# sndels/yuki

Measured on AMD Instinct MI355X. Metric: Mray/s (primary+secondary), Path integrator @1080p, higher is better.
Workload: dtype f32; 1 GPU; cfg3: city 40x20 displaced icospheres, 1,024,012 triangles, SAH BVH (max_shapes_in_node 1), Path 8 bounces, Stratified 8x8, 1920x1080; triangles=1024012, spp=64, max_depth=8, tiles=8160, partition=single GPU, frames_in_flight=2

## Files before the change

### yuki_amd/csrc/yk_kernels.h

```cpp
#pragma once
#include <hip/hip_runtime.h>

#include "yk_device.h"

namespace yk {

unsigned trace_block_size();
unsigned trace_spill_depth();
unsigned trace_top_nodes();
unsigned trace_top_nodes_any();
unsigned packet_blocks_per_cu();
void launch_trace_closest_packet(hipStream_t s, unsigned grid, const DevScene& sc, const float4* rayO, const float4* rayD, const unsigned* count_ptr,
                                 unsigned* head, int* hit_tri, unsigned long long* ray_counter, const float4* lean_origin = nullptr, CancelRef cancel = CancelRef{nullptr, nullptr});
void launch_trace_any_packet(hipStream_t s, unsigned grid, const DevScene& sc, const ShadowQueue& q, unsigned char* vis, unsigned long long* shadow_counter,
                             CancelRef cancel = CancelRef{nullptr, nullptr});
unsigned trace_blocks_per_cu();

void launch_pixel_table(hipStream_t s, const yk_tile* tiles, const uint32_t* tile_offset, uint32_t n_tiles, uint32_t n_pixels, uint32_t* pixel_xy,
                        const uint16_t* tile_sample = nullptr, uint32_t* pixel_sample = nullptr);
void launch_pixel_table_one(hipStream_t s, const yk_tile& tile, uint32_t n_pixels, uint32_t* pixel_xy, uint32_t tile_sample, uint32_t* pixel_sample);
void launch_raygen(hipStream_t s, const DevCamera& cam, const RenderParams& prm, const uint32_t* pixel_xy, const uint32_t* pixel_sample, uint64_t work0,
                   uint32_t n, PathBuffers out, float4* sample_buf, unsigned* count, float4* lean_origin = nullptr, const uint4* pixel_aux = nullptr);
void launch_pixel_sampler(hipStream_t s, const SamplerCfg& cfg, const uint32_t* pixel_xy, uint32_t n_pixels, uint4* pixel_aux);
void launch_raygen_user(hipStream_t s, const RenderParams& prm, const float* o, const float* d, const uint16_t* pixel, const uint32_t* sample_index,
                        uint32_t dimension, uint32_t n, PathBuffers out, float4* sample_buf, uint32_t* pixel_xy, unsigned* ctrl);
void launch_trace_closest(hipStream_t s, unsigned grid, const DevScene& sc, const float4* rayO, const float4* rayD, const float* t_max_opt,
                          const unsigned* count_ptr, unsigned* head, int* hit_tri, float4* hit_out, uint4* stats_out, uint2* spill,
                          unsigned spill_stride, unsigned* ctrl, unsigned long long* ray_counter, const unsigned* cancel_host = nullptr);
void launch_whitted(hipStream_t s, unsigned grid, const DevScene& sc, const RenderParams& prm, const uint32_t* pixel_xy, const uint32_t* sample_index_tab,
                    PathBuffers cur, uint32_t n, float4* sample_buf, uint2* spill, unsigned spill_stride, unsigned* ctrl, unsigned long long* counters);
unsigned whitted_max_depth();
void launch_path_debug(hipStream_t s, unsigned grid, const DevScene& sc, const RenderParams& prm, const uint32_t* pixel_xy, const uint32_t* sample_index_tab,
                       PathBuffers cur, uint32_t n, float4* sample_buf, uint32_t* out_counts, float4* out_rays, unsigned ray_cap, uint32_t* out_n_rays,
                       float min_len, uint2* spill, unsigned spill_stride, unsigned* ctrl);
void launch_trace_any(hipStream_t s, unsigned grid, const DevScene& sc, const ShadowQueue& q, unsigned char* vis, uint2* spill, unsigned spill_stride,
                      unsigned* ctrl, unsigned long long* shadow_counter, const unsigned* cancel_host = nullptr);
void launch_shade(hipStream_t s, unsigned grid, const DevScene& sc, const RenderParams& prm, const uint32_t* pixel_xy, const uint32_t* sample_index_tab,
                  PathBuffers cur, PathBuffers nxt, const BounceQueues& q, unsigned split_delta, unsigned reorder, unsigned block_slots, unsigned sid_base,
                  const float4* lean_origin);
void launch_accumulate(hipStream_t s, unsigned grid, const RenderParams& prm, PathBuffers cur, const BounceQueues& q, unsigned nl, float4* sample_buf,
                       unsigned first, unsigned sid_base);
void launch_resolve(hipStream_t s, const float4* sample_buf, uint32_t n_pixels, uint32_t spp, float* out_rgb);
void launch_resolve_passes(hipStream_t s, const float4* sample_buf, uint32_t n_pixels, uint32_t n_passes, float* out_rgb, size_t pass_stride);
void launch_film_scatter(hipStream_t s, const uint32_t* pixel_xy, uint32_t n_pixels, const float* tile_rgb, uint32_t res_x, float* film_rgb, int accumulate,
                         uint32_t n_passes = 1, size_t pass_stride = 0);
void launch_debug_shade(hipStream_t s, const DevScene& sc, uint32_t integrator, PathBuffers cur, const int* hit_tri, const uint4* stats, uint32_t n,
                        float4* sample_buf);
void launch_guides(hipStream_t s, const DevScene& sc, PathBuffers cur, const int* hit_tri, uint32_t n, const uint32_t* pixel_xy, uint32_t res_x, float4* guides);
void launch_guides_ids(hipStream_t s, const DevScene& sc, PathBuffers cur, const int* hit_tri, uint32_t n, const uint32_t* pixel_xy, uint32_t res_x, float4* guides, uint4* ids);
void launch_ad_fold_samples(hipStream_t s, const uint32_t* pixel_xy, uint32_t n, const float4* sample_buf, uint32_t n_passes, uint32_t res_x, float* film_sum,
                            void* stats);
void launch_device_math(hipStream_t s, int fn, size_t n, const float* a, const float* b, float* out);
void launch_sampler_sequence(hipStream_t s, const SamplerCfg& cfg, uint32_t px, uint32_t py, uint32_t sample_index, const uint8_t* dims, size_t n_draws,
                             float* out);
void launch_light_test(hipStream_t s, const DevLight& L, int index, size_t n, const float* p, const float* ng, const float* u, float* out);
void launch_bsdf_test(hipStream_t s, const Material& m, size_t n, const float* ng, const float* ns, const float* dpdu, const float* wo,
                      const float* wi_or_u, int sample, float* out);
void launch_surface_test(hipStream_t s, const DevScene& sc, size_t n, const float4* rayO, const float4* rayD, const int* hit_word, int route, float* out);
void launch_pack_rays(hipStream_t s, size_t n, const float* o, const float* d, float4* rayO, float4* rayD);
void launch_pack_shadow_rays(hipStream_t s, size_t n, const float* o, const float* d, const float* t_max, const int* area_light, float4* shO,
                             float4* shD);
void launch_unpack_rays(hipStream_t s, size_t n, const float4* rayO, const float4* rayD, float* o, float* d);

}
```

### yuki_amd/csrc/yk_kernels.hip

```cpp
#include <hip/hip_runtime.h>

#include "yk_device.h"
#include "yk_geom.h"
#include "yk_kernels.h"
#include "yk_path_state.h"
#include "yk_rng.h"
#include "yk_shade.h"
#include "yk_shade_queue.h"
#include "yk_wave.h"

namespace yk {

__global__ void k_pixel_table(const yk_tile* tiles, const uint32_t* tile_offset, uint32_t n_tiles, uint32_t n_pixels,
                              uint32_t* pixel_xy, const uint16_t* tile_sample, uint32_t* pixel_sample) {
    uint32_t i = blockIdx.x * blockDim.x + threadIdx.x;
    if (i >= n_pixels) return;
    uint32_t lo = 0, hi = n_tiles;
    while (hi - lo > 1) {
        uint32_t mid = (lo + hi) >> 1;
        if (tile_offset[mid] <= i)
            lo = mid;
        else
            hi = mid;
    }
// ... 6 lines not shown
}

__global__ void k_pixel_table_one(yk_tile t, uint32_t n_pixels, uint32_t* pixel_xy, uint32_t tile_sample, uint32_t* pixel_sample) {
    uint32_t i = blockIdx.x * blockDim.x + threadIdx.x;
    if (i >= n_pixels) return;
    uint32_t w = (uint32_t)t.x1 - t.x0;
    pixel_xy[i] = (t.x0 + i % w) | ((t.y0 + i / w) << 16);
    if (pixel_sample) pixel_sample[i] = tile_sample;
}

__global__ void k_pixel_sampler(SamplerCfg cfg, const uint32_t* pixel_xy, uint32_t n_pixels, uint4* pixel_aux) {
    uint32_t i = blockIdx.x * blockDim.x + threadIdx.x;
    if (i >= n_pixels) return;
    const uint32_t xy = pixel_xy[i];
    const PixelSampler ps = pixel_sampler(cfg, xy & 0xffffu, xy >> 16);
    pixel_aux[i] = make_uint4((unsigned)ps.stream, (unsigned)(ps.stream >> 32), ps.hash0, 0u);
}

__device__ __forceinline__ void camera_ray(const DevCamera& cam, float fx, float fy, V3& o, V3& d) {
    V3 p_camera = xf_point(cam.r2c, V3{fx, fy, 0.0f});
    V3 dir = normalize(p_camera);
    o = xf_point(cam.c2w, V3{0.0f, 0.0f, 0.0f});
    d = xf_vector(cam.c2w, dir);
}

__global__ void k_raygen(DevCamera cam, RenderParams prm, const uint32_t* pixel_xy, const uint32_t* pixel_sample, uint64_t work0, uint32_t n,
                         PathBuffers out, float4* sample_buf, unsigned* count, float4* lean_origin, const uint4* pixel_aux) {
    uint32_t i = blockIdx.x * blockDim.x + threadIdx.x;
    if (cancel_raised(prm.cancel)) return;
    if (i == 0) *count = n;
    if (i >= n) return;
    const uint32_t w = (uint32_t)(work0 + i);
    uint32_t pix, ks;
    split_sample_id(w, prm.spe, pix, ks);
    const uint32_t s = (pixel_sample ? pixel_sample[pix] : prm.sample_base) + ks;
    uint32_t xy = pixel_xy[pix];
    uint32_t px = xy & 0xffffu, py = xy >> 16;
    SamplerState st;
    float ux, uy;
    if (pixel_aux) {
        const uint4 a = pixel_aux[pix];
        PixelSampler ps;
        ps.stream = (u64)a.x | ((u64)a.y << 32);
        ps.hash0 = a.z;
        st = sampler_start_camera(prm.sampler, ps, px, py, s, ux, uy);
    } else {
        st = sampler_start(prm.sampler, px, py, s, 0);
        sampler_get_2d(prm.sampler, st, ux, uy);
    }
    V3 o, d;
    camera_ray(cam, (float)px + ux, (float)py + uy, o, d);
    path_store_camera(out, i, o, d, w, st, lean_origin, i == 0);
    if (prm.integrator != YK_INTEGRATOR_PATH || prm.max_depth == 0) sample_buf[w] = make_float4(0.0f, 0.0f, 0.0f, 0.0f);
}

__global__ void k_raygen_user(RenderParams prm, const float* ray_o, const float* ray_d, const uint16_t* pixel, const uint32_t* sample_index,
                              uint32_t dimension, uint32_t n, PathBuffers out, float4* sample_buf, uint32_t* pixel_xy, unsigned* count) {
    uint32_t i = blockIdx.x * blockDim.x + threadIdx.x;
    if (i == 0) *count = n;
    if (i >= n) return;
    uint32_t px = pixel[2 * i], py = pixel[2 * i + 1];
    pixel_xy[i] = px | (py << 16);
    SamplerState st = sampler_start(prm.sampler, px, py, sample_index[i], dimension);
    if (prm.sampler.kind == 1) st.dimension = dimension;
    path_store_camera(out, i, ld3(ray_o, i), ld3(ray_d, i), i, st, nullptr, false);
    if (prm.integrator != YK_INTEGRATOR_PATH || prm.max_depth == 0) sample_buf[i] = make_float4(0.0f, 0.0f, 0.0f, 0.0f);
}

#ifdef YK_SHADE_PROFILE
#include "../../tools/micro/shade_profile.h"
#else
#define YK_PROF_DECL
#define YK_PROF_STAMP(k)
#define YK_PROF_FLUSH
#endif

template <int BLOCK, int CAP, int CAPQ>
__global__ __launch_bounds__(BLOCK, SHADE_MIN_WAVES) void k_shade(DevScene sc, RenderParams prm, const uint32_t* pixel_xy, const uint32_t* sample_index_tab,
                                                                  PathBuffers cur, PathBuffers nxt, BounceQueues q, ShadeArgs a,
                                                                  const float4* __restrict__ lean_origin) {
    static_assert(sizeof(ShadeStaging<CAP, CAPQ>) <= 53296, "k_shade: more LDS than the measured 53296 bytes per block (42 granules = 53760 cost the third block per CU)");
    __shared__ ShadeStaging<CAP, CAPQ> stg;
    const unsigned win_iters = min(a.win_max, max(1u, *q.count / (BLOCK * a.block_slots)));
    ShadeQueue<BLOCK, CAP, CAPQ> sq(stg, q, nxt, sc, a.split_delta);
    const unsigned n = sq.begin(prm.cancel);
    const unsigned WIN = win_iters * BLOCK;
    const unsigned n_win = (n + WIN - 1) / WIN;
    YK_PROF_DECL
    for (unsigned w = blockIdx.x; w < n_win; w += gridDim.x) {
        const unsigned wbase = w * WIN;
        YK_PROF_STAMP(0)
        const unsigned n_sub = a.reorder ? sort_window<BLOCK>(stg, q.hit, wbase, win_iters, n) : plain_window<BLOCK>(wbase, win_iters, n);
        for (unsigned sub = 0; sub < n_sub; ++sub) {
            const unsigned i = wbase + window_offset<BLOCK>(stg, a.reorder, sub);
            const bool valid = i < n;
            YK_PROF_STAMP(1)
            sq.room_for_iteration();
            PathState ps = path_inert();
            SamplerState st = sampler_inert();
            PathVertex v = vertex_inert();
            bool hit = false;
            if (valid) {
                ps = path_load(cur, i, lean_origin);
                st = path_sampler(prm, pixel_xy, sample_index_tab, ps);
                const int tri = q.hit[i];
                hit = tri >= 0;
                if (hit) vertex_setup(sc, (uint32_t)tri & YK_HIT_PRIM_MASK, ps.o, ps.d, v);
            }
            YK_PROF_STAMP(2)
            unsigned vword = 0u;
            for (unsigned l = 0; l < sq.nl; ++l) {
                NeeSample ne = nee_none();
                if (valid && hit) ne = vertex_light(sc, prm, st, l, v);
                sq.stage_shadow(ne, valid, i, l, vword);
            }
            sq.store_verdicts(valid, i, vword);
            YK_PROF_STAMP(3)
            bool alive = false;
            PathWords next = PathWords{make_float4(0, 0, 0, 0), make_float4(0, 0, 0, 0), make_float4(0, 0, 0, 0), make_uint4(0, 0, 0, 0)};
            if (valid) {
                unsigned kind = YK_PEND_MISS;
                RGB term = RGB{0, 0, 0};
                if (!hit) {
                    term = vertex_miss_term(sc, ps.beta);
                } else {
                    const VertexEnd e = vertex_finish(sc, prm, st, v, ps.beta, ps.bounces, ps.specular);
                    term = e.term;
                    kind = e.kind;
                    alive = e.alive;
                    if (e.sampled) {
                        ps.o = e.no;
                        ps.d = e.wi;
                        ps.dimension = st.dimension;
                        ps.rng = st.rng;
                        next = path_pack(ps);
                    }
                }
                q.pend[i] = pend_pack(term, kind, ps.sid - a.sid_base);
            }
            YK_PROF_STAMP(4)
            sq.stage_survivor(alive, next);
            YK_PROF_STAMP(5)
        }
        if (a.reorder) __syncthreads();
    }
    YK_PROF_FLUSH
    sq.finish();
}

__global__ void k_accumulate(RenderParams prm, PathBuffers cur, BounceQueues q, unsigned nl, float4* sample_buf, unsigned first, unsigned sid_base) {
    const unsigned n = cancel_raised(prm.cancel) ? 0u : *q.count;
    for (unsigned i = blockIdx.x * blockDim.x + threadIdx.x; i < n; i += gridDim.x * blockDim.x) {
        float4 p = q.pend[i];
        const unsigned kind = pend_kind(p);
        const unsigned sid = sid_base + pend_slot(p);
        RGB beta = RGB{1.0f, 1.0f, 1.0f};
        if (!first && !(kind & YK_PEND_MISS)) beta = path_beta(cur.thru[i]);
        RGB L = RGB{0.0f, 0.0f, 0.0f};
        if (!first) {
            const float4 acc = sample_buf[sid];
            L = RGB{acc.x, acc.y, acc.z};
        }
        RGB radiance = RGB{0.0f, 0.0f, 0.0f};
        if (!(kind & YK_PEND_MISS)) {
            const unsigned vs = YK_VIS_STRIDE(nl);
            const unsigned vword = vs == 4u ? reinterpret_cast<const unsigned*>(q.vis)[i] : 0u;
            for (unsigned l = 0; l < nl; ++l) {
// ... 70 lines not shown

__global__ void k_debug_shade(DevScene sc, uint32_t integrator, PathBuffers cur, const int* hit_tri, const uint4* stats, uint32_t n,
                              float4* sample_buf) {
    uint32_t i = blockIdx.x * blockDim.x + threadIdx.x;
    if (i >= n) return;
    const float4 rd = cur.rayD[i];
    int tri = hit_tri[i];
    RGB c = RGB{0.0f, 0.0f, 0.0f};
    if (integrator == YK_INTEGRATOR_BVH_INTERSECTIONS) {
        uint4 s = stats[i];
        c = RGB{(float)s.x, (float)s.y, tri >= 0 ? (float)s.y : 0.0f};
    } else if (tri >= 0 && integrator == YK_INTEGRATOR_SHADING_UVS) {
        Surface sf = hit_surface_prim(sc, (uint32_t)tri & YK_HIT_PRIM_MASK, f4_xyz(cur.rayO[i]), f4_xyz(rd), true);
        c = RGB{sf.u, sf.v, 0.0f};
    } else if (tri >= 0) {
        Surface sf = hit_surface_prim(sc, (uint32_t)tri & YK_HIT_PRIM_MASK, f4_xyz(cur.rayO[i]), f4_xyz(rd));
        V3 nn = integrator == YK_INTEGRATOR_GEOMETRY_NORMALS ? sf.n : sf.ns;
        c = RGB{nn.x, nn.y, nn.z} / 2.0f + 0.5f;
    }
    sample_buf[path_sample_id(rd)] = make_float4(c.r, c.g, c.b, 0.0f);
}

template <bool IDS>
__global__ void k_guides(DevScene sc, PathBuffers cur, const int* hit_tri, uint32_t n, const uint32_t* pixel_xy, uint32_t res_x, float4* guides, uint4* ids) {
    uint32_t i = blockIdx.x * blockDim.x + threadIdx.x;
    if (i >= n) return;
    const float4 rd = cur.rayD[i];
    const uint32_t xy = pixel_xy[path_sample_id(rd)];
    const size_t px = (size_t)(xy >> 16) * res_x + (xy & 0xffffu);
    const int tri = hit_tri[i];
    float4 a = make_float4(0.0f, 0.0f, 0.0f, 0.0f), b = a;
    uint4 id = make_uint4(YK_SURFACE_NONE, 0u, 0u, 0u);
    if (tri >= 0) {
        float t = 0.0f;
        const Surface sf = hit_surface_prim(sc, (uint32_t)tri & YK_HIT_PRIM_MASK, f4_xyz(cur.rayO[i]), f4_xyz(rd), sc.texels != nullptr, &t, IDS ? &id : nullptr);
        a = make_float4(sf.ns.x, sf.ns.y, sf.ns.z, 1.0f);
        b = make_float4(sf.p.x, sf.p.y, sf.p.z, t);
    }
    if (!IDS || guides) {
        guides[2 * px] = a;
        guides[2 * px + 1] = b;
    }
    if (IDS && ids) ids[px] = id;
}

#ifdef YK_SHADE_PROFILE
}
extern "C" int yk_debug_shade_profile(unsigned long long* out8, int reset) {
    unsigned long long zero[8] = {0, 0, 0, 0, 0, 0, 0, 0};
    (void)hipDeviceSynchronize();
    int rc = (int)hipMemcpyFromSymbol(out8, HIP_SYMBOL(yk::yk_shade_prof), sizeof(zero));
    if (reset) rc |= (int)hipMemcpyToSymbol(HIP_SYMBOL(yk::yk_shade_prof), zero, sizeof(zero));
    return rc;
}
namespace yk {
#endif

static inline unsigned blocks_for(size_t n, unsigned bs) { return (unsigned)((n + bs - 1) / bs); }

void launch_pixel_table(hipStream_t s, const yk_tile* tiles, const uint32_t* tile_offset, uint32_t n_tiles, uint32_t n_pixels, uint32_t* pixel_xy,
                        const uint16_t* tile_sample, uint32_t* pixel_sample) {
    if (!n_pixels) return;
    hipLaunchKernelGGL(k_pixel_table, dim3(blocks_for(n_pixels, 256)), dim3(256), 0, s, tiles, tile_offset, n_tiles, n_pixels, pixel_xy, tile_sample,
                       pixel_sample);
}
void launch_pixel_table_one(hipStream_t s, const yk_tile& tile, uint32_t n_pixels, uint32_t* pixel_xy, uint32_t tile_sample, uint32_t* pixel_sample) {
    if (!n_pixels) return;
    hipLaunchKernelGGL(k_pixel_table_one, dim3(blocks_for(n_pixels, 256)), dim3(256), 0, s, tile, n_pixels, pixel_xy, tile_sample, pixel_sample);
}
void launch_pixel_sampler(hipStream_t s, const SamplerCfg& cfg, const uint32_t* pixel_xy, uint32_t n_pixels, uint4* pixel_aux) {
    if (!n_pixels) return;
    hipLaunchKernelGGL(k_pixel_sampler, dim3(blocks_for(n_pixels, 256)), dim3(256), 0, s, cfg, pixel_xy, n_pixels, pixel_aux);
}
void launch_raygen(hipStream_t s, const DevCamera& cam, const RenderParams& prm, const uint32_t* pixel_xy, const uint32_t* pixel_sample, uint64_t work0,
                   uint32_t n, PathBuffers out, float4* sample_buf, unsigned* count, float4* lean_origin, const uint4* pixel_aux) {
    hipLaunchKernelGGL(k_raygen, dim3(blocks_for(n, 256)), dim3(256), 0, s, cam, prm, pixel_xy, pixel_sample, work0, n, out, sample_buf, count, lean_origin, pixel_aux);
}
void launch_raygen_user(hipStream_t s, const RenderParams& prm, const float* o, const float* d, const uint16_t* pixel, const uint32_t* sample_index,
                        uint32_t dimension, uint32_t n, PathBuffers out, float4* sample_buf, uint32_t* pixel_xy, unsigned* ctrl) {
    hipLaunchKernelGGL(k_raygen_user, dim3(blocks_for(n, 256)), dim3(256), 0, s, prm, o, d, pixel, sample_index, dimension, n, out, sample_buf,
                       pixel_xy, ctrl);
}
void launch_shade(hipStream_t s, unsigned grid, const DevScene& sc, const RenderParams& prm, const uint32_t* pixel_xy, const uint32_t* sample_index_tab,
                  PathBuffers cur, PathBuffers nxt, const BounceQueues& q, unsigned split_delta, unsigned reorder, unsigned block_slots, unsigned sid_base,
                  const float4* lean_origin) {
    const ShadeArgs a{split_delta, reorder, (unsigned)SHADE_WIN, block_slots, sid_base};
    hipLaunchKernelGGL((k_shade<256, SHADE_CAP, SHADE_CAPQ>), dim3(grid), dim3(256), 0, s, sc, prm, pixel_xy, sample_index_tab, cur, nxt, q, a, lean_origin);
}
void launch_accumulate(hipStream_t s, unsigned grid, const RenderParams& prm, PathBuffers cur, const BounceQueues& q, unsigned nl, float4* sample_buf,
                       unsigned first, unsigned sid_base) {
    hipLaunchKernelGGL(k_accumulate, dim3(grid), dim3(256), 0, s, prm, cur, q, nl, sample_buf, first, sid_base);
}
void launch_resolve(hipStream_t s, const float4* sample_buf, uint32_t n_pixels, uint32_t spp, float* out_rgb) {
    if (!n_pixels) return;
    hipLaunchKernelGGL(k_resolve, dim3(blocks_for(n_pixels, 256)), dim3(256), 0, s, sample_buf, n_pixels, spp, out_rgb);
}
void launch_resolve_passes(hipStream_t s, const float4* sample_buf, uint32_t n_pixels, uint32_t n_passes, float* out_rgb, size_t pass_stride) {
    if (!n_pixels) return;
    hipLaunchKernelGGL(k_resolve_passes, dim3(blocks_for((size_t)n_pixels * n_passes, 256)), dim3(256), 0, s, sample_buf, n_pixels, n_passes, out_rgb, pass_stride);
}
void launch_film_scatter(hipStream_t s, const uint32_t* pixel_xy, uint32_t n_pixels, const float* tile_rgb, uint32_t res_x, float* film_rgb, int accumulate,
                         uint32_t n_passes, size_t pass_stride) {
    if (!n_pixels) return;
    hipLaunchKernelGGL(k_film_scatter, dim3(blocks_for(n_pixels, 256)), dim3(256), 0, s, pixel_xy, n_pixels, tile_rgb, res_x, film_rgb, accumulate, n_passes, pass_stride);
}
void launch_debug_shade(hipStream_t s, const DevScene& sc, uint32_t integrator, PathBuffers cur, const int* hit_tri, const uint4* stats, uint32_t n,
                        float4* sample_buf) {
    hipLaunchKernelGGL(k_debug_shade, dim3(blocks_for(n, 256)), dim3(256), 0, s, sc, integrator, cur, hit_tri, stats, n, sample_buf);
}
void launch_guides(hipStream_t s, const DevScene& sc, PathBuffers cur, const int* hit_tri, uint32_t n, const uint32_t* pixel_xy, uint32_t res_x, float4* guides) {
    hipLaunchKernelGGL(k_guides<false>, dim3(blocks_for(n, 256)), dim3(256), 0, s, sc, cur, hit_tri, n, pixel_xy, res_x, guides, (uint4*)nullptr);
}
void launch_guides_ids(hipStream_t s, const DevScene& sc, PathBuffers cur, const int* hit_tri, uint32_t n, const uint32_t* pixel_xy, uint32_t res_x, float4* guides, uint4* ids) {
    hipLaunchKernelGGL(k_guides<true>, dim3(blocks_for(n, 256)), dim3(256), 0, s, sc, cur, hit_tri, n, pixel_xy, res_x, guides, ids);
}

}
```

### yuki_amd/csrc/yk_render.cpp

```cpp
#include <hip/hip_runtime.h>

#include <algorithm>
#include <chrono>
#include <cstdio>
#include <cstdlib>
#include <cstring>
#include <memory>
#include <mutex>
#include <string>
#include <thread>
#include <vector>

#include "yk_adaptive.h"
#include "yk_albedo.h"
#include "yk_film_call.h"
#include "yk_render_plan.h"
#include "yk_staging.h"
#ifdef YK_EXPERIMENT_SORT
#include "../../tools/micro/ray_sort_experiment.h"
#endif
#ifdef YK_EXPERIMENT_GRAPH
#include "../../tools/micro/graph_replay_experiment.h"
#endif

// ... 45 lines not shown
    p.thru = ws.path[which][2].as<float4>();
    p.rngs = ws.path[which][3].as<uint4>();
    return p;
}

static BounceQueues bounce_queues(WorkSet& ws, unsigned b) {
    unsigned* bc = ws.ctrl.as<unsigned>() + YK_CTRL_BOUNCE(b);
    BounceQueues q;
    q.hit = ws.hit.as<int>();
    q.pend = ws.pend.as<float4>();
    q.shC = ws.shC.as<float4>();
    q.vis = ws.vis.as<unsigned char>();
    q.area = ShadowQueue{ws.shO.as<float4>(), ws.shD.as<float4>(), ws.shq.as<unsigned>(), bc + YK_CTRL_SHQ, bc + YK_CTRL_HEAD + 1};
    q.delta = ShadowQueue{ws.shO2.as<float4>(), ws.shD2.as<float4>(), ws.shq2.as<unsigned>(), bc + YK_CTRL_SHQ2, bc + YK_CTRL_HEAD + 2};
    q.count = bc;
    q.next_count = bc + YK_CTRL_STRIDE;
    q.closest_head = bc + YK_CTRL_HEAD;
    return q;
}

yk_status make_params(yk_context* ctx, const yk_sampler_desc* smp, const yk_integrator_desc* integ, RenderParams& prm) {
    if (!smp || !integ) return fail(ctx, YK_ERR_INVALID_ARGUMENT, "null sampler/integrator");
    std::memset(&prm, 0, sizeof(prm));
    prm.sampler.kind = smp->kind;
    prm.sampler.nx = smp->nx;
    prm.sampler.ny = smp->kind == YK_SAMPLER_UNIFORM ? 1 : smp->ny;
    prm.sampler.jitter = smp->jitter;
    prm.sampler.seed = smp->seed;
    if (smp->kind > 1 || prm.sampler.nx == 0 || prm.sampler.ny == 0) return fail(ctx, YK_ERR_INVALID_ARGUMENT, "bad sampler");
    uint64_t spp = (uint64_t)prm.sampler.nx * prm.sampler.ny;
    if (spp > 0xFFFFu) return fail(ctx, YK_ERR_INVALID_ARGUMENT, "samples per pixel exceed u16 (integrators/mod.rs:139)");
    prm.sampler.spp = (unsigned)spp;
    prm.spe = (unsigned)spp;
    prm.max_depth = integ->max_depth;
    prm.has_clamp = integ->has_clamp;
    prm.clamp = integ->indirect_clamp;
    prm.integrator = integ->kind;
    if (integ->kind == YK_INTEGRATOR_WHITTED && integ->max_depth > whitted_max_depth())
        return fail(ctx, YK_ERR_UNSUPPORTED, "Whitted: max_depth above 16 is not supported on the device");
    if (integ->kind > YK_INTEGRATOR_SHADING_UVS) return fail(ctx, YK_ERR_INVALID_ARGUMENT, "bad integrator kind");
    return YK_OK;
}


bool packet_kernel_traces_bounce(const yk_context* ctx, const yk_scene* scene, unsigned b) {
    return b < (unsigned)ctx->packet_bounces && scene->bvh->depth <= 64;
}

void run_bounces(yk_context* ctx, WorkSet& ws, hipStream_t st, const yk_scene* scene, const RenderParams& prm, const uint32_t* pixel_xy,
                        const uint32_t* sample_index_tab, float4* sample_buf, KernelTimer& kt, unsigned long long* counters, bool coherent,
                        uint32_t n_paths, uint32_t sid_base, bool lean_camera_bounce, uint32_t* n_shadow_launches) {
    unsigned* ctrl = ws.ctrl.as<unsigned>();
    unsigned* errblk = error_block(ctx);
    const DevScene ds = dev_scene_for(scene, n_paths);
    auto fit = [](unsigned full, uint64_t items) { return (unsigned)std::min<uint64_t>(full, std::max<uint64_t>(1, (items + 255) / 256)); };
    const uint64_t n_shadow_max = (uint64_t)n_paths * std::max(1u, scene->n_lights);
    const unsigned tg = fit(trace_grid(ctx), n_paths), tg_any = fit(trace_grid(ctx), n_shadow_max);
    const unsigned pg_full = (unsigned)ctx->n_cu * packet_blocks_per_cu();
    const unsigned pg = fit(pg_full, n_paths), pg_any = fit(pg_full, n_shadow_max);
    static const unsigned shade_bpc = std::getenv("YK_SHADE_BPC") ? (unsigned)std::atoi(std::getenv("YK_SHADE_BPC")) : 256u;
    const unsigned sg = fit((unsigned)ctx->n_cu * shade_bpc, n_paths);
    const unsigned spill_stride = trace_grid(ctx) * trace_block_size();
    unsigned cur = 0;
    const bool overlap = ctx->overlap_shadow != 0 && ws.side != nullptr;
    hipStream_t sb = overlap ? ws.side : st;
    for (unsigned b = 0; b < prm.max_depth; ++b) {
        PathBuffers pc = path_buffers(ws, (int)cur), pn = path_buffers(ws, (int)(cur ^ 1u));
        const bool packet = coherent && packet_kernel_traces_bounce(ctx, scene, b);
        const float4* lean_origin = (b == 0 && lean_camera_bounce) ? reinterpret_cast<const float4*>(ctrl + YK_CTRL_CAM_O) : nullptr;
        const bool packet_shadow = coherent && b < (unsigned)ctx->packet_shadow_bounces && scene->bvh->depth <= 64 && scene->n_delta_lights > 0;
        const bool split = packet_shadow && scene->n_lights > scene->n_delta_lights;
        const bool all_delta = packet_shadow && !split;
        BounceQueues q = bounce_queues(ws, b);
        int e = kt.begin(st);
        if (packet)
            launch_trace_closest_packet(st, pg, ds, lean_origin ? nullptr : pc.rayO, pc.rayD, q.count, q.closest_head, q.hit, counters, lean_origin, prm.cancel);
        else {
            launch_trace_closest(st, tg, ds, pc.rayO, pc.rayD, nullptr, q.count, q.closest_head, q.hit, nullptr, nullptr,
                                 ws.spill.as<uint2>(), spill_stride, errblk, counters, prm.cancel.host);
        }
        kt.end(e, 0, st);
        if (overlap && b > 0) (void)hipStreamWaitEvent(st, ws.ev_acc, 0);
        e = kt.begin(st);
        launch_shade(st, sg, ds, prm, pixel_xy, sample_index_tab, pc, pn, q, split ? 1u : 0u, (b > 0 && ctx->shade_reorder) ? 1u : 0u, 3u * (unsigned)ctx->n_cu,
                     sid_base, lean_origin);
        kt.end(e, 2, st);
#ifdef YK_EXPERIMENT_SORT
        YK_SORT_AFTER_SHADE
#endif
        if (overlap) {
            (void)hipEventRecord(ws.ev_shade, st);
            (void)hipStreamWaitEvent(sb, ws.ev_shade, 0);
        }
        e = kt.begin(sb);
        uint2* any_spill = (overlap ? ws.spill_side : ws.spill).as<uint2>();
        if (all_delta) {
            launch_trace_any_packet(sb, pg_any, ds, q.area, q.vis, counters + 1, prm.cancel);
        } else {
            launch_trace_any(sb, tg_any, ds, q.area, q.vis, any_spill, spill_stride, errblk, counters + 1, prm.cancel.host);
            if (split && n_shadow_launches) ++*n_shadow_launches;
            if (split)
                launch_trace_any_packet(sb, pg_any, ds, q.delta, q.vis, counters + 1, prm.cancel);
        }
        kt.end(e, 1, sb);
        if (n_shadow_launches) ++*n_shadow_launches;
        launch_accumulate(sb, sg, prm, pc, q, ds.n_lights, sample_buf, b == 0 ? 1u : 0u, sid_base);
        if (overlap) (void)hipEventRecord(ws.ev_acc, sb);
        if (kt.on && std::getenv("YK_DEBUG_BOUNCES")) {
            unsigned h[YK_CTRL_STRIDE + 1];
            (void)hipStreamSynchronize(st);
            (void)hipStreamSynchronize(sb);
            (void)hipMemcpy(h, q.count, sizeof(h), hipMemcpyDeviceToHost);
            float tt = 0, ts = 0, th = 0;
            (void)hipEventElapsedTime(&tt, ctx->ev_pool[kt.spans[0].back().first], ctx->ev_pool[kt.spans[0].back().second]);
            (void)hipEventElapsedTime(&ts, ctx->ev_pool[kt.spans[1].back().first], ctx->ev_pool[kt.spans[1].back().second]);
            (void)hipEventElapsedTime(&th, ctx->ev_pool[kt.spans[2].back().first], ctx->ev_pool[kt.spans[2].back().second]);
            std::fprintf(stderr, "bounce %u: rays %u trace %.3f ms (%.0f Mray/s) | shadow rays %u %.3f ms (%.0f Mray/s) | shade %.3f ms | survivors %u\n", b, h[0],
                         tt, h[0] / (tt * 1e3), h[YK_CTRL_SHQ] + h[YK_CTRL_SHQ2], ts, (h[YK_CTRL_SHQ] + h[YK_CTRL_SHQ2]) / (ts * 1e3), th, h[YK_CTRL_STRIDE]);
        }
        cur ^= 1u;
    }
    if (overlap) (void)hipStreamWaitEvent(st, ws.ev_acc, 0);
}

static double now_ms() { return std::chrono::duration<double, std::milli>(std::chrono::steady_clock::now().time_since_epoch()).count(); }
static const bool g_debug_cancel = std::getenv("YK_DEBUG_CANCEL") != nullptr;

static void raise_cancel(yk_context* ctx, bool from_render_thread = true) {
    if (!ctx->cancel_host) return;
    const double t0 = g_debug_cancel ? now_ms() : 0.0;
    ctx->cancel_raised.store(true, std::memory_order_release);
    __atomic_store_n(ctx->cancel_host, 1u, __ATOMIC_RELEASE);
    if (from_render_thread && !ctx->cancel_stream) ctx->want_cancel_stream = true;
    if (from_render_thread && ctx->cancel_stream && ctx->counters.p)
        (void)hipMemcpyAsync(error_block(ctx) + YK_CTRL_CANCELLED, ctx->cancel_host + 16, 4, hipMemcpyHostToDevice, ctx->cancel_stream);
    if (g_debug_cancel) std::fprintf(stderr, "[yk cancel] raise: %s, %.3f ms\n", ctx->cancel_stream ? "host word + device word" : "host word only (first interruption)", now_ms() - t0);
}

static yk_status clear_cancel(yk_context* ctx) {
    if (!ctx->cancel_host || !ctx->cancel_raised.load(std::memory_order_acquire)) return YK_OK;
    HIP_TRY(ctx, hipStreamSynchronize(ctx->stream));
    if (ctx->cancel_stream) HIP_TRY(ctx, hipStreamSynchronize(ctx->cancel_stream));
    for (WorkSet& w : ctx->ws) {
        if (w.stream && w.stream != ctx->stream) HIP_TRY(ctx, hipStreamSynchronize(w.stream));
        if (w.side) HIP_TRY(ctx, hipStreamSynchronize(w.side));
    }
    __atomic_store_n(ctx->cancel_host, 0u, __ATOMIC_RELEASE);
    ctx->cancel_raised.store(false, std::memory_order_release);
    if (ctx->want_cancel_stream && !ctx->cancel_stream) {
        if (hipStreamCreateWithFlags(&ctx->cancel_stream, hipStreamNonBlocking) != hipSuccess) ctx->cancel_stream = nullptr;
        ctx->want_cancel_stream = false;
    }
    return YK_OK;
}

static bool poll_until(yk_context* ctx, hipEvent_t done, yk_cancel_fn cancel, void* user) {
    while (hipEventQuery(done) == hipErrorNotReady) {
        if (cancel(user)) {
            raise_cancel(ctx);
            return true;
        }
        std::this_thread::sleep_for(std::chrono::microseconds(100));
    }
    return false;
}
static bool wait_polling(yk_context* ctx, hipEvent_t done, hipStream_t st, yk_cancel_fn cancel, void* user) {
    const bool fired = cancel ? poll_until(ctx, done, cancel, user) : false;
    (void)hipStreamSynchronize(st);
// ... 913 lines not shown
```

### yuki_amd/csrc/yk_shade_queue.h

```cpp
#pragma once
#include "yk_device.h"
#include "yk_path_state.h"
#include "yk_shade.h"
#include "yk_wave.h"

#ifndef SHADE_CAP
#define SHADE_CAP 335
#endif
#ifndef SHADE_CAPQ
#define SHADE_CAPQ 768
#endif
#ifndef SHADE_WIN
#define SHADE_WIN 8
#endif
#ifndef SHADE_MIN_WAVES
#define SHADE_MIN_WAVES 3
#endif

namespace yk {

template <int CAP, int CAPQ> struct ShadeStaging {
    float4 pO[CAP], pD[CAP], pT[CAP];
    uint4 pR[CAP];
    float4 qO[CAPQ], qD[CAPQ];
    unsigned qS[CAPQ];
    unsigned fill_p, fill_q, gbase;
    unsigned q_delta;
    unsigned cancel;
    unsigned bucket[8];
    unsigned short order[SHADE_WIN * 256];
};

struct ShadeArgs {
    unsigned split_delta;
    unsigned reorder;
    unsigned win_max;
    unsigned block_slots;
    unsigned sid_base;
};

__device__ __forceinline__ unsigned block_append(bool want, unsigned* lds_fill) {
    unsigned long long mask = __ballot(want);
    unsigned total = (unsigned)__popcll(mask);
    unsigned prefix = (unsigned)__popcll(mask & ((1ull << lane_id()) - 1ull));
    unsigned base = 0;
    if (total && lane_id() == 0) base = atomicAdd(lds_fill, total);
    base = __shfl(base, 0);
    return base + prefix;
}

template <int BLOCK, class Staging>
__device__ __forceinline__ unsigned sort_window(Staging& stg, const int* hit_tri, unsigned wbase, unsigned win_iters, unsigned n) {
    if (threadIdx.x < 8) stg.bucket[threadIdx.x] = 0;
    __syncthreads();
    unsigned key[SHADE_WIN], rank[SHADE_WIN];
#pragma unroll
    for (int k = 0; k < SHADE_WIN; ++k) {
        const unsigned i0 = wbase + k * BLOCK + threadIdx.x;
        const bool in = (unsigned)k < win_iters && i0 < n;
        const int t = in ? hit_tri[i0] : -1;
        key[k] = !in ? 7u : (t < 0 ? 6u : ((unsigned)t >> YK_HIT_KIND_SHIFT));
    }
#pragma unroll
    for (int k = 0; k < SHADE_WIN; ++k) {
        rank[k] = 0;
        if ((unsigned)k >= win_iters) continue;
        for (unsigned q = 0; q < 8; ++q) {
            const unsigned long long m = __ballot(key[k] == q);
            if (m == 0ull) continue;
            unsigned b0 = 0;
            if (lane_id() == 0) b0 = atomicAdd(&stg.bucket[q], (unsigned)__popcll(m));
            b0 = __shfl(b0, 0);
            if (key[k] == q) rank[k] = b0 + (unsigned)__popcll(m & ((1ull << lane_id()) - 1ull));
        }
    }
    __syncthreads();
    unsigned first[8], n_sub;
    {
        unsigned acc = 0;
        for (unsigned q = 0; q < 8; ++q) {
            first[q] = acc;
            acc += stg.bucket[q];
        }
        n_sub = (acc - stg.bucket[7] + BLOCK - 1) / BLOCK;
    }
#pragma unroll
    for (int k = 0; k < SHADE_WIN; ++k)
        if ((unsigned)k < win_iters) stg.order[first[key[k]] + rank[k]] = (unsigned short)(k * BLOCK + threadIdx.x);
    __syncthreads();
    return n_sub;
}
template <int BLOCK> __device__ __forceinline__ unsigned plain_window(unsigned wbase, unsigned win_iters, unsigned n) {
    const unsigned left = n - wbase;
    return left >= win_iters * BLOCK ? win_iters : (left + BLOCK - 1) / BLOCK;
}
template <int BLOCK, class Staging> __device__ __forceinline__ unsigned window_offset(const Staging& stg, unsigned reorder, unsigned sub) {
    return reorder ? (unsigned)stg.order[sub * BLOCK + threadIdx.x] : sub * BLOCK + threadIdx.x;
}

template <int BLOCK, int CAP, int CAPQ> struct ShadeQueue {
    ShadeStaging<CAP, CAPQ>& stg;
    const BounceQueues& q;
    const PathBuffers& nxt;
    const DevScene& sc;
    const unsigned nl, split_delta;
    const bool per_iter;

    __device__ __forceinline__ ShadeQueue(ShadeStaging<CAP, CAPQ>& stg_, const BounceQueues& q_, const PathBuffers& nxt_, const DevScene& sc_, unsigned split_delta_)
        : stg(stg_), q(q_), nxt(nxt_), sc(sc_), nl(sc_.n_lights), split_delta(split_delta_), per_iter(!split_delta_ && BLOCK * sc_.n_lights <= (unsigned)CAPQ) {}

    __device__ __forceinline__ unsigned begin(const CancelRef& cancel) {
        if (threadIdx.x == 0) {
            stg.fill_p = 0;
            stg.fill_q = 0;
            stg.q_delta = 0;
            stg.cancel = cancel_raised(cancel) ? 1u : 0u;
        }
        __syncthreads();
        return __builtin_amdgcn_readfirstlane((int)stg.cancel) ? 0u : *q.count;
    }

    __device__ __forceinline__ void flush_q(unsigned fill, unsigned delta) {
        if (threadIdx.x == 0) stg.gbase = atomicAdd(delta ? q.delta.count : q.area.count, fill);
        __syncthreads();
        const unsigned gb = stg.gbase;
        float4* dO = delta ? q.delta.O : q.area.O;
        float4* dD = delta ? q.delta.D : q.area.D;
        unsigned* dS = delta ? q.delta.slot : q.area.slot;
        for (unsigned k = threadIdx.x; k < fill; k += BLOCK) {
            dO[gb + k] = stg.qO[k];
            dD[gb + k] = stg.qD[k];
            dS[gb + k] = stg.qS[k];
        }
        __syncthreads();
        if (threadIdx.x == 0) stg.fill_q = 0;
        __syncthreads();
    }
    __device__ __forceinline__ void flush_p(unsigned fill) {
        if (threadIdx.x == 0) stg.gbase = atomicAdd(q.next_count, fill);
        __syncthreads();
        const unsigned gb = stg.gbase;
        for (unsigned k = threadIdx.x; k < fill; k += BLOCK) {
            nxt.rayO[gb + k] = stg.pO[k];
            nxt.rayD[gb + k] = stg.pD[k];
            nxt.thru[gb + k] = stg.pT[k];
            nxt.rngs[gb + k] = stg.pR[k];
        }
        __syncthreads();
        if (threadIdx.x == 0) stg.fill_p = 0;
        __syncthreads();
    }

    __device__ __forceinline__ void room_for_iteration() {
        if (!per_iter) return;
        __syncthreads();
        const unsigned fq = stg.fill_q, fp = stg.fill_p, staged = stg.q_delta;
        __syncthreads();
        if (fq && fq + BLOCK * nl > CAPQ) flush_q(fq, staged);
        if (fp + BLOCK > CAP) flush_p(fp);
    }
    __device__ __forceinline__ void room_for_light(unsigned l) {
        if (per_iter) return;
        __syncthreads();
        const unsigned f = stg.fill_q, staged = stg.q_delta;
        const unsigned delta = (split_delta && sc.lights[l].kind != YK_LIGHT_RECT) ? 1u : 0u;
        __syncthreads();
        if (f && (staged != delta || f + BLOCK > CAPQ)) flush_q(f, staged);
        if (threadIdx.x == 0) stg.q_delta = delta;
    }
    __device__ __forceinline__ void room_for_survivor() {
        if (per_iter) return;
        __syncthreads();
        const unsigned f = stg.fill_p;
        __syncthreads();
        if (f + BLOCK > CAP) flush_p(f);
    }

    __device__ __forceinline__ void stage_shadow(const NeeSample& ne, bool valid, unsigned i, unsigned l, unsigned& vword) {
        const unsigned vs = YK_VIS_STRIDE(nl);
        const unsigned slot = i * nl + l, vslot = i * vs + l;
        const bool want = ne.want;
        if (vs == 4u)
            vword |= (want ? 1u : 0u) << (8u * l);
        else if (valid)
            q.vis[vslot] = want ? 1 : 0;
        room_for_light(l);
        const unsigned k = block_append(want, &stg.fill_q);
        if (want) {
            stg.qO[k] = make_float4(ne.so.x, ne.so.y, ne.so.z, YK_SHADOW_T_MAX);
            stg.qD[k] = make_float4(ne.sd.x, ne.sd.y, ne.sd.z, __uint_as_float((unsigned)ne.al));
            stg.qS[k] = vslot;
            q.shC[slot] = make_float4(ne.contrib.r, ne.contrib.g, ne.contrib.b, 0.0f);
        }
    }
    __device__ __forceinline__ void store_verdicts(bool valid, unsigned i, unsigned vword) {
        if (YK_VIS_STRIDE(nl) == 4u && valid) reinterpret_cast<unsigned*>(q.vis)[i] = vword;
    }

    __device__ __forceinline__ void stage_survivor(bool alive, const PathWords& w) {
        room_for_survivor();
        const unsigned j = block_append(alive, &stg.fill_p);
        if (alive) {
            stg.pO[j] = w.O;
            stg.pD[j] = w.D;
            stg.pT[j] = w.T;
            stg.pR[j] = w.R;
        }
    }

    __device__ __forceinline__ void finish() {
        __syncthreads();
        const unsigned fq = stg.fill_q, fp = stg.fill_p;
        if (fq) flush_q(fq, stg.q_delta);
        if (fp) flush_p(fp);
    }
};

}
```

Before: 2283 Mray/s.

## Split shade shadow staging into per-class LDS regions with merged flushes

The shade kernel's shadow-ray staging buffer is split into separate area and delta regions sized by a host-computed plan, so the kernel no longer flushes whenever the light class changes. All three queues (survivors, area, delta) are flushed together in one barrier round, with their atomics issued from different waves. Survivor staging capacity drops from 335 to 256, which shrinks LDS use but can force survivor flushes more often. The per-iteration decision mode now depends on the light count fitting the region slots even when delta lights are split.

```diff
diff --git a/yuki_amd/csrc/yk_kernels.h b/yuki_amd/csrc/yk_kernels.h
--- a/yuki_amd/csrc/yk_kernels.h
+++ b/yuki_amd/csrc/yk_kernels.h
@@ -36,8 +36,8 @@
 void launch_trace_any(hipStream_t s, unsigned grid, const DevScene& sc, const ShadowQueue& q, unsigned char* vis, uint2* spill, unsigned spill_stride,
                       unsigned* ctrl, unsigned long long* shadow_counter, const unsigned* cancel_host = nullptr);
 void launch_shade(hipStream_t s, unsigned grid, const DevScene& sc, const RenderParams& prm, const uint32_t* pixel_xy, const uint32_t* sample_index_tab,
-                  PathBuffers cur, PathBuffers nxt, const BounceQueues& q, unsigned split_delta, unsigned reorder, unsigned block_slots, unsigned sid_base,
-                  const float4* lean_origin);
+                  PathBuffers cur, PathBuffers nxt, const BounceQueues& q, unsigned split_delta, unsigned n_area_lights, unsigned reorder,
+                  unsigned block_slots, unsigned sid_base, const float4* lean_origin);
 void launch_accumulate(hipStream_t s, unsigned grid, const RenderParams& prm, PathBuffers cur, const BounceQueues& q, unsigned nl, float4* sample_buf,
                        unsigned first, unsigned sid_base);
 void launch_resolve(hipStream_t s, const float4* sample_buf, uint32_t n_pixels, uint32_t spp, float* out_rgb);
diff --git a/yuki_amd/csrc/yk_kernels.hip b/yuki_amd/csrc/yk_kernels.hip
--- a/yuki_amd/csrc/yk_kernels.hip
+++ b/yuki_amd/csrc/yk_kernels.hip
@@ -112,7 +112,7 @@
     static_assert(sizeof(ShadeStaging<CAP, CAPQ>) <= 53296, "k_shade: more LDS than the measured 53296 bytes per block (42 granules = 53760 cost the third block per CU)");
     __shared__ ShadeStaging<CAP, CAPQ> stg;
     const unsigned win_iters = min(a.win_max, max(1u, *q.count / (BLOCK * a.block_slots)));
-    ShadeQueue<BLOCK, CAP, CAPQ> sq(stg, q, nxt, sc, a.split_delta);
+    ShadeQueue<BLOCK, CAP, CAPQ> sq(stg, q, nxt, sc, a);
     const unsigned n = sq.begin(prm.cancel);
     const unsigned WIN = win_iters * BLOCK;
     const unsigned n_win = (n + WIN - 1) / WIN;
@@ -349,9 +349,10 @@
                        pixel_xy, ctrl);
 }
 void launch_shade(hipStream_t s, unsigned grid, const DevScene& sc, const RenderParams& prm, const uint32_t* pixel_xy, const uint32_t* sample_index_tab,
-                  PathBuffers cur, PathBuffers nxt, const BounceQueues& q, unsigned split_delta, unsigned reorder, unsigned block_slots, unsigned sid_base,
-                  const float4* lean_origin) {
-    const ShadeArgs a{split_delta, reorder, (unsigned)SHADE_WIN, block_slots, sid_base};
+                  PathBuffers cur, PathBuffers nxt, const BounceQueues& q, unsigned split_delta, unsigned n_area_lights, unsigned reorder,
+                  unsigned block_slots, unsigned sid_base, const float4* lean_origin) {
+    const ShadeRegions regions = shade_regions(sc.n_lights, split_delta ? n_area_lights : sc.n_lights, (unsigned)SHADE_CAPQ, 256u);
+    const ShadeArgs a{split_delta, regions, reorder, (unsigned)SHADE_WIN, block_slots, sid_base};
     hipLaunchKernelGGL((k_shade<256, SHADE_CAP, SHADE_CAPQ>), dim3(grid), dim3(256), 0, s, sc, prm, pixel_xy, sample_index_tab, cur, nxt, q, a, lean_origin);
 }
 void launch_accumulate(hipStream_t s, unsigned grid, const RenderParams& prm, PathBuffers cur, const BounceQueues& q, unsigned nl, float4* sample_buf,
diff --git a/yuki_amd/csrc/yk_render.cpp b/yuki_amd/csrc/yk_render.cpp
--- a/yuki_amd/csrc/yk_render.cpp
+++ b/yuki_amd/csrc/yk_render.cpp
@@ -151,8 +151,8 @@
         kt.end(e, 0, st);
         if (overlap && b > 0) (void)hipStreamWaitEvent(st, ws.ev_acc, 0);
         e = kt.begin(st);
-        launch_shade(st, sg, ds, prm, pixel_xy, sample_index_tab, pc, pn, q, split ? 1u : 0u, (b > 0 && ctx->shade_reorder) ? 1u : 0u, 3u * (unsigned)ctx->n_cu,
-                     sid_base, lean_origin);
+        launch_shade(st, sg, ds, prm, pixel_xy, sample_index_tab, pc, pn, q, split ? 1u : 0u, scene->n_lights - scene->n_delta_lights,
+                     (b > 0 && ctx->shade_reorder) ? 1u : 0u, 3u * (unsigned)ctx->n_cu, sid_base, lean_origin);
         kt.end(e, 2, st);
 #ifdef YK_EXPERIMENT_SORT
         YK_SORT_AFTER_SHADE
diff --git a/yuki_amd/csrc/yk_shade_queue.h b/yuki_amd/csrc/yk_shade_queue.h
--- a/yuki_amd/csrc/yk_shade_queue.h
+++ b/yuki_amd/csrc/yk_shade_queue.h
@@ -2,10 +2,11 @@
 #include "yk_device.h"
 #include "yk_path_state.h"
 #include "yk_shade.h"
+#include "yk_shade_regions.h"
 #include "yk_wave.h"
 
 #ifndef SHADE_CAP
-#define SHADE_CAP 335
+#define SHADE_CAP 256
 #endif
 #ifndef SHADE_CAPQ
 #define SHADE_CAPQ 768
@@ -24,8 +25,9 @@
     uint4 pR[CAP];
     float4 qO[CAPQ], qD[CAPQ];
     unsigned qS[CAPQ];
-    unsigned fill_p, fill_q, gbase;
-    unsigned q_delta;
+    unsigned fill_p;
+    unsigned fill_q[2];
+    unsigned gbase_p, gbase_q[2];
     unsigned cancel;
     unsigned bucket[8];
     unsigned short order[SHADE_WIN * 256];
@@ -33,6 +35,7 @@
 
 struct ShadeArgs {
     unsigned split_delta;
+    ShadeRegions regions;
     unsigned reorder;
     unsigned win_max;
     unsigned block_slots;
@@ -99,81 +102,93 @@
 }
 
 template <int BLOCK, int CAP, int CAPQ> struct ShadeQueue {
+    static_assert(CAP >= BLOCK, "the survivor staging holds an iteration");
+    static_assert(CAPQ % BLOCK == 0 && CAPQ >= 2 * BLOCK, "shade_regions deals whole blocks, at least one per class");
+    static_assert(BLOCK >= 192, "flush: threads 0, 64 and 128 reserve");
     ShadeStaging<CAP, CAPQ>& stg;
     const BounceQueues& q;
     const PathBuffers& nxt;
     const DevScene& sc;
     const unsigned nl, split_delta;
     const bool per_iter;
-
-    __device__ __forceinline__ ShadeQueue(ShadeStaging<CAP, CAPQ>& stg_, const BounceQueues& q_, const PathBuffers& nxt_, const DevScene& sc_, unsigned split_delta_)
-        : stg(stg_), q(q_), nxt(nxt_), sc(sc_), nl(sc_.n_lights), split_delta(split_delta_), per_iter(!split_delta_ && BLOCK * sc_.n_lights <= (unsigned)CAPQ) {}
+    const unsigned delta_base;
+    const unsigned full_area, full_delta;
+
+    __device__ __forceinline__ ShadeQueue(ShadeStaging<CAP, CAPQ>& stg_, const BounceQueues& q_, const PathBuffers& nxt_, const DevScene& sc_, const ShadeArgs& a)
+        : stg(stg_), q(q_), nxt(nxt_), sc(sc_), nl(sc_.n_lights), split_delta(a.split_delta), per_iter(a.regions.one_decision != 0u),
+          delta_base(a.regions.delta_base),
+          full_area(room_left(a.regions.area_cap, per_iter ? a.regions.need_area : (unsigned)BLOCK)),
+          full_delta(room_left(a.regions.delta_cap, per_iter ? a.regions.need_delta : (unsigned)BLOCK)) {}
+    static __device__ __forceinline__ unsigned room_left(unsigned cap, unsigned need) { return cap > need ? cap - need : 0u; }
+
+    static __device__ __forceinline__ unsigned uniform(unsigned v) { return (unsigned)__builtin_amdgcn_readfirstlane((int)v); }
+    __device__ __forceinline__ unsigned light_class(unsigned l) const { return (split_delta && sc.lights[l].kind != YK_LIGHT_RECT) ? 1u : 0u; }
 
     __device__ __forceinline__ unsigned begin(const CancelRef& cancel) {
         if (threadIdx.x == 0) {
             stg.fill_p = 0;
-            stg.fill_q = 0;
-            stg.q_delta = 0;
+            stg.fill_q[0] = 0;
+            stg.fill_q[1] = 0;
             stg.cancel = cancel_raised(cancel) ? 1u : 0u;
         }
         __syncthreads();
-        return __builtin_amdgcn_readfirstlane((int)stg.cancel) ? 0u : *q.count;
-    }
-
-    __device__ __forceinline__ void flush_q(unsigned fill, unsigned delta) {
-        if (threadIdx.x == 0) stg.gbase = atomicAdd(delta ? q.delta.count : q.area.count, fill);
-        __syncthreads();
-        const unsigned gb = stg.gbase;
-        float4* dO = delta ? q.delta.O : q.area.O;
-        float4* dD = delta ? q.delta.D : q.area.D;
-        unsigned* dS = delta ? q.delta.slot : q.area.slot;
+        return uniform(stg.cancel) ? 0u : *q.count;
+    }
+
+    __device__ __forceinline__ void copy_q(const ShadowQueue& dst, unsigned base, unsigned fill, unsigned gb) {
         for (unsigned k = threadIdx.x; k < fill; k += BLOCK) {
-            dO[gb + k] = stg.qO[k];
-            dD[gb + k] = stg.qD[k];
-            dS[gb + k] = stg.qS[k];
-        }
-        __syncthreads();
-        if (threadIdx.x == 0) stg.fill_q = 0;
-        __syncthreads();
-    }
-    __device__ __forceinline__ void flush_p(unsigned fill) {
-        if (threadIdx.x == 0) stg.gbase = atomicAdd(q.next_count, fill);
-        __syncthreads();
-        const unsigned gb = stg.gbase;
-        for (unsigned k = threadIdx.x; k < fill; k += BLOCK) {
-            nxt.rayO[gb + k] = stg.pO[k];
-            nxt.rayD[gb + k] = stg.pD[k];
-            nxt.thru[gb + k] = stg.pT[k];
-            nxt.rngs[gb + k] = stg.pR[k];
-        }
-        __syncthreads();
-        if (threadIdx.x == 0) stg.fill_p = 0;
+            dst.O[gb + k] = stg.qO[base + k];
+            dst.D[gb + k] = stg.qD[base + k];
+            dst.slot[gb + k] = stg.qS[base + k];
+        }
+    }
+    __device__ __forceinline__ void flush(unsigned fp, unsigned fa, unsigned fd) {
+        if (threadIdx.x == 0 && fp) stg.gbase_p = atomicAdd(q.next_count, fp);
+        if (threadIdx.x == 64 && fa) stg.gbase_q[0] = atomicAdd(q.area.count, fa);
+        if (threadIdx.x == 128 && fd) stg.gbase_q[1] = atomicAdd(q.delta.count, fd);
+        __syncthreads();
+        if (fp) {
+            const unsigned gb = stg.gbase_p;
+            for (unsigned k = threadIdx.x; k < fp; k += BLOCK) {
+                nxt.rayO[gb + k] = stg.pO[k];
+                nxt.rayD[gb + k] = stg.pD[k];
+                nxt.thru[gb + k] = stg.pT[k];
+                nxt.rngs[gb + k] = stg.pR[k];
+            }
+        }
+        if (fa) copy_q(q.area, 0u, fa, stg.gbase_q[0]);
+        if (fd) copy_q(q.delta, delta_base, fd, stg.gbase_q[1]);
+        if (threadIdx.x == 0 && fp) stg.fill_p = 0;
+        if (threadIdx.x == 64 && fa) stg.fill_q[0] = 0;
+        if (threadIdx.x == 128 && fd) stg.fill_q[1] = 0;
         __syncthreads();
     }
 
     __device__ __forceinline__ void room_for_iteration() {
         if (!per_iter) return;
         __syncthreads();
-        const unsigned fq = stg.fill_q, fp = stg.fill_p, staged = stg.q_delta;
-        __syncthreads();
-        if (fq && fq + BLOCK * nl > CAPQ) flush_q(fq, staged);
-        if (fp + BLOCK > CAP) flush_p(fp);
-    }
-    __device__ __forceinline__ void room_for_light(unsigned l) {
+        const unsigned fp = uniform(stg.fill_p), fa = uniform(stg.fill_q[0]), fd = uniform(stg.fill_q[1]);
+        const unsigned np = fp + BLOCK > CAP ? fp : 0u;
+        const unsigned na = fa > full_area ? fa : 0u;
+        const unsigned nd = fd > full_delta ? fd : 0u;
+        if (np | na | nd)
+            flush(np, na, nd);
+        else
+            __syncthreads();
+    }
+    __device__ __forceinline__ void room_for_light(unsigned c) {
         if (per_iter) return;
         __syncthreads();
-        const unsigned f = stg.fill_q, staged = stg.q_delta;
-        const unsigned delta = (split_delta && sc.lights[l].kind != YK_LIGHT_RECT) ? 1u : 0u;
-        __syncthreads();
-        if (f && (staged != delta || f + BLOCK > CAPQ)) flush_q(f, staged);
-        if (threadIdx.x == 0) stg.q_delta = delta;
+        const unsigned f = uniform(stg.fill_q[c]);
+        __syncthreads();
+        if (f > (c ? full_delta : full_area)) flush(0u, c ? 0u : f, c ? f : 0u);
     }
     __device__ __forceinline__ void room_for_survivor() {
         if (per_iter) return;
         __syncthreads();
-        const unsigned f = stg.fill_p;
-        __syncthreads();
-        if (f + BLOCK > CAP) flush_p(f);
+        const unsigned f = uniform(stg.fill_p);
+        __syncthreads();
+        if (f + BLOCK > CAP) flush(f, 0u, 0u);
     }
 
     __device__ __forceinline__ void stage_shadow(const NeeSample& ne, bool valid, unsigned i, unsigned l, unsigned& vword) {
@@ -184,8 +199,9 @@
             vword |= (want ? 1u : 0u) << (8u * l);
         else if (valid)
             q.vis[vslot] = want ? 1 : 0;
-        room_for_light(l);
-        const unsigned k = block_append(want, &stg.fill_q);
+        const unsigned c = light_class(l);
+        room_for_light(c);
+        const unsigned k = (c ? delta_base : 0u) + block_append(want, &stg.fill_q[c]);
         if (want) {
             stg.qO[k] = make_float4(ne.so.x, ne.so.y, ne.so.z, YK_SHADOW_T_MAX);
             stg.qD[k] = make_float4(ne.sd.x, ne.sd.y, ne.sd.z, __uint_as_float((unsigned)ne.al));
@@ -210,9 +226,8 @@
 
     __device__ __forceinline__ void finish() {
         __syncthreads();
-        const unsigned fq = stg.fill_q, fp = stg.fill_p;
-        if (fq) flush_q(fq, stg.q_delta);
-        if (fp) flush_p(fp);
+        const unsigned fp = uniform(stg.fill_p), fa = uniform(stg.fill_q[0]), fd = uniform(stg.fill_q[1]);
+        if (fp | fa | fd) flush(fp, fa, fd);
     }
 };
 
diff --git a/yuki_amd/csrc/yk_shade_regions.h b/yuki_amd/csrc/yk_shade_regions.h
--- /dev/null
+++ b/yuki_amd/csrc/yk_shade_regions.h
@@ -0,0 +1,44 @@
+#pragma once
+
+#if defined(__HIPCC__) || defined(__CUDACC__)
+#define YK_REGIONS_FN __host__ __device__ inline
+#else
+#define YK_REGIONS_FN inline
+#endif
+
+namespace yk {
+
+struct ShadeRegions {
+    unsigned area_base, area_cap;
+    unsigned delta_base, delta_cap;
+    unsigned need_area, need_delta;
+    unsigned one_decision;
+};
+
+YK_REGIONS_FN constexpr ShadeRegions shade_regions(unsigned nl, unsigned n_area, unsigned capq, unsigned block) {
+    const unsigned na = n_area < nl ? n_area : nl, nd = nl - na;
+    const unsigned slots = capq / block;
+    unsigned area_slots = 0;
+    if (nd == 0)
+        area_slots = slots;
+    else if (na == 0)
+        area_slots = 0;
+    else if (nl <= slots)
+        area_slots = na;
+    else {
+        area_slots = (unsigned)(((unsigned long long)slots * na) / nl);
+        if (area_slots < 1u) area_slots = 1u;
+        if (area_slots > slots - 1u) area_slots = slots - 1u;
+    }
+    ShadeRegions r{};
+    r.area_base = 0u;
+    r.area_cap = area_slots * block;
+    r.delta_base = r.area_cap;
+    r.delta_cap = nd ? (nl <= slots && na ? nd * block : (slots - area_slots) * block) : 0u;
+    r.need_area = na * block;
+    r.need_delta = nd * block;
+    r.one_decision = (nl <= slots) ? 1u : 0u;
+    return r;
+}
+
+}
```

Result: no change. 2267 Mray/s (-0.7%).
